# tmuird/VAEUNET

Hardware: AMD Instinct MI355X
Metric: images/sec (whole node) at 3x512x512 bs=8/GPU; Dice parity vs CPU ref (higher is better)
Workload: dtype bf16; 1 GPU; UNet(3,2) train step (fwd+CombinedLoss+bwd+clip+AdamW), random-init weights; image=3x512x512, batch_per_gpu=8, global_batch=8, parallelism=dp1, execution=hipgraph-replay, wgrad_side_stream=False

## Files before the change

### include/vaeunet.h

```cpp
#ifndef VAEUNET_H
#define VAEUNET_H
#include <stdint.h>
#ifdef __cplusplus
extern "C" {
#endif

typedef struct VuGather {
  const void* src[3];
  int64_t stride[3];
  int32_t cend[3];
  int32_t nsrc;
  int32_t C;
  int32_t N, H, W;
  int32_t Hs, Ws;
  int32_t R, S;
  int32_t sy, sx, dy, dx, oy, ox;
} VuGather;

typedef struct VuGemmFwd {
  VuGather a;
  const void* b;
  int64_t ldb;
  int32_t ncol;
  int32_t out_mode;
// ... 216 lines not shown
                    int dtype, void* stream);
int vu_attn_gate_fwd(const float* q, const float* st, const void* x,
                     int64_t xs, int64_t P, int C, float* pmap, void* out,
                     int64_t os, int dtype, void* stream);
int vu_attn_gate_bwd(const void* dout, int64_t dos, const void* x, int64_t xs,
                     const float* pmap, int64_t P, int C, void* dx,
                     int64_t dxs, float* dqpre, int dtype, void* stream);
int64_t vu_attn_psi_bwd_workspace_bytes(int64_t P, int F);
int vu_attn_psi_bwd(const void* ug, const void* ux, int64_t P, int F,
                    const float* sg, const float* tg, const float* sx,
                    const float* tx, const float* wpsi, const float* dq,
                    void* ds, float* dwpsi, float* dbpsi, int accumulate,
                    float* workspace, int dtype, void* stream);
int64_t vu_attn_psi_bwd_blocks(int64_t P);
int vu_attn_psi_bwd_bnb_ok(int F);
int vu_attn_psi_bwd_bnb(const void* ug, const void* ux, int64_t P, int F,
                        const float* sg, const float* tg, const float* sx,
                        const float* tx, const float* wpsi, const float* dq,
                        void* ds, float* dwpsi, float* dbpsi, int accumulate,
                        float* workspace, const float* mean_g, const float* invstd_g,
                        const float* mean_x, const float* invstd_x, float* bnb_g,
                        float* bnb_x, int dtype, void* stream);

int vu_pointwise_fwd(const void* x, int64_t xs, int64_t P, int C, int J,
                     const float* w, const float* b, float* y, int64_t ys,
                     int dtype, void* stream);
int64_t vu_pointwise_bwd_workspace_bytes(int64_t P, int C, int J);
int vu_pointwise_bwd(const void* x, int64_t xs, const float* dy, int64_t dys,
                     int64_t P, int C, int J, const float* w, void* dx,
                     int64_t dxs, float* dw, float* db, int accumulate,
                     float* workspace, int dtype, void* stream);
int vu_pointwise_bn_fwd(const void* x, int64_t xs, int64_t P, int C, int J,
                        const float* bn_scale, const float* bn_shift, const float* w,
                        const float* b, float* y, int64_t ys, int dtype, void* stream);
int64_t vu_pointwise_bn_bwd_blocks(int64_t P);
int vu_pointwise_bn_bwd(const void* x, int64_t xs, const float* bn_coef, int64_t coef_stride,
                        const float* dy, int64_t dys, int64_t P, int C, int J, const float* w,
                        void* dx, int64_t dxs, float* dw, float* db, int accumulate,
                        float* workspace, float* bnb, int dtype, void* stream);

int64_t vu_loss_workspace_bytes(void);
int vu_bce_dice_fwd2(const float* logits, const float* target, int64_t n,
                     double* sums, float smooth, float w_bce, float w_dice,
                     float* loss, float* parts, double* workspace,
                     void* stream);
int vu_bce_dice_fwd(const float* logits, const float* target, int64_t n,
// ... 197 lines not shown
```

### vaeunet_amd/_lib.py

```python
import ctypes as C
import os

import torch

_HERE = os.path.dirname(os.path.abspath(__file__))
LIB_PATH = os.path.join(_HERE, "libvaeunet_hip.so")
if os.environ.get("VU_LIB_PATH"):
    LIB_PATH = os.environ["VU_LIB_PATH"]

F32, BF16 = 0, 1

_p = C.c_void_p
_i = C.c_int
_l = C.c_int64
_f = C.c_float


class VuGather(C.Structure):
    _fields_ = [("src", _p * 3), ("stride", _l * 3), ("cend", C.c_int32 * 3),
                ("nsrc", C.c_int32), ("C", C.c_int32),
                ("N", C.c_int32), ("H", C.c_int32), ("W", C.c_int32),
                ("Hs", C.c_int32), ("Ws", C.c_int32), ("R", C.c_int32), ("S", C.c_int32),
                ("sy", C.c_int32), ("sx", C.c_int32), ("dy", C.c_int32), ("dx", C.c_int32),
                ("oy", C.c_int32), ("ox", C.c_int32)]
# ... 108 lines not shown
    "vu_chan_sum": (_i, [_p, _l, _i, _i, _i, _i, _i, _i, _i, _i, _p, _i, _p, _i, _p]),
    "vu_copy": (_i, [_p, _l, _i, _p, _l, _i, _l, _i, _i, _p]),
    "vu_zero": (_i, [_p, _l, _l, _i, _i, _p]),
    "vu_gpu_delay": (_i, [_i, _p]),
    "vu_zero_insert2": (_i, [_p, _l, _i, _i, _i, _i, _p, _l, _i, _i, _i, _p]),
    "vu_input_pack": (_i, [_p, _l, _l, _l, _l, _i, _i, _i, _i, _i, _p, _i, _p]),
    "vu_maxpool2_fwd": (_i, [_p, _l, _i, _i, _i, _i, _p, _l, _i, _p]),
    "vu_maxpool2_bwd": (_i, [_p, _l, _p, _l, _i, _i, _i, _i, _p, _l, _p, _l, _i, _p]),
    "vu_bn_apply_maxpool2": (_i, [_p, _l, _p, _l, _p, _l, _i, _i, _i, _i, _p, _p, _i, _i, _p]),
    "vu_upsample_fwd": (_i, [_p, _l, _i, _i, _i, _i, _p, _l, _i, _i, _i, _i, _i, _i, _i, _p]),
    "vu_upsample_bwd": (_i, [_p, _l, _i, _i, _i, _i, _p, _l, _i, _i, _i, _i, _i, _i, _i, _i,
                             _p]),
    "vu_attn_tile_rows": (_l, []),
    "vu_attn_psi_fwd": (_i, [_p, _p, _l, _i, _p, _p, _p, _p, _p, _p, _p, _p, _p, _l, _i, _p]),
    "vu_attn_gate_fwd": (_i, [_p, _p, _p, _l, _l, _i, _p, _p, _l, _i, _p]),
    "vu_attn_gate_bwd": (_i, [_p, _l, _p, _l, _p, _l, _i, _p, _l, _p, _i, _p]),
    "vu_attn_psi_bwd_workspace_bytes": (_l, [_l, _i]),
    "vu_attn_psi_bwd_blocks": (_l, [_l]),
    "vu_attn_psi_bwd_bnb_ok": (_i, [_i]),
    "vu_attn_psi_bwd_bnb": (_i, [_p, _p, _l, _i, _p, _p, _p, _p, _p, _p, _p, _p, _p, _i, _p, _p, _p, _p, _p, _p, _p,
                                 _i, _p]),
    "vu_attn_psi_bwd": (_i, [_p, _p, _l, _i, _p, _p, _p, _p, _p, _p, _p, _p, _p, _i, _p, _i,
                             _p]),
    "vu_pointwise_fwd": (_i, [_p, _l, _l, _i, _i, _p, _p, _p, _l, _i, _p]),
    "vu_pointwise_bwd_workspace_bytes": (_l, [_l, _i, _i]),
    "vu_pointwise_bn_fwd": (_i, [_p, _l, _l, _i, _i, _p, _p, _p, _p, _p, _l, _i, _p]),
    "vu_pointwise_bn_bwd_blocks": (_l, [_l]),
    "vu_pointwise_bn_bwd": (_i, [_p, _l, _p, _l, _p, _l, _l, _i, _i, _p, _p, _l, _p, _p, _i, _p, _p, _i, _p]),
    "vu_pointwise_bwd": (_i, [_p, _l, _p, _l, _l, _i, _i, _p, _p, _l, _p, _p, _i, _p, _i, _p]),
    "vu_loss_workspace_bytes": (_l, []),
    "vu_bce_dice_fwd2": (_i, [_p, _p, _l, _p, _f, _f, _f, _p, _p, _p, _p]),
    "vu_bce_dice_bwd": (_i, [_p, _p, _l, _p, _f, _f, _f, _p, _p, _p]),
    "vu_kl_free_bits2": (_i, [_p, _p, _i, _i, _f, _p, _p, _p, _p, _p]),
    "vu_sumsq": (_i, [_p, _l, _p, _p, _p]),
    "vu_dice_score": (_i, [_p, _p, _l, _f, _p, _p, _p, _p]),
    "vu_seg_counts_workspace_bytes": (_l, [_l]),
    "vu_seg_counts": (_i, [_p, _i, C.POINTER(_l), _i, _i, _p, _i, C.POINTER(_l), _i, _i, _i, _i, _i, _i, _p, _i, _p,
                           _p, _p]),
    "vu_seg_metrics": (_i, [_p, _i, _i, C.c_double, _p, _p, _i, _p, _p]),
    "vu_mt_chunk_elems": (_l, []),
    "vu_mt_grad_norm": (_i, [_p, _i, _l, _f, _p, _p, _p, _p]),
    "vu_mt_scale_grads": (_i, [_p, _i, _l, _p, _p]),
    "vu_mt_adamw": (_i, [_p, _i, _l, _f, _f, _f, _f, _f, _p, _p]),
    "vu_mt_adamw_dev": (_i, [_p, _i, _l, C.c_double, C.c_double, C.c_double, C.c_double, C.c_double, _p, _i,
                             _p]),
    "vu_mt_adamw_dev_scaled": (_i, [_p, _i, _l, C.c_double, C.c_double, C.c_double, C.c_double, C.c_double, _p,
# ... 77 lines not shown
```

### vaeunet_amd/csrc/attention.hip

```cpp
#include "host.h"

namespace {

constexpr int TILE = 256;

template <int CTRL>
VU_DEV float dpp_f(float v) {
  return __int_as_float(__builtin_amdgcn_update_dpp(0, __float_as_int(v), CTRL, 0xf, 0xf, false));
}

VU_DEV void vec8_tie(Vec8<bf16_t>& v) { asm volatile("" : "+v"(v.v)); }
VU_DEV void vec8_tie(Vec8<float>& v) { asm volatile("" : "+v"(v.a), "+v"(v.b)); }

VU_DEV float group_sum(float v, int lpp) {
  if (lpp >= 2) v += dpp_f<0xB1>(v);
  if (lpp >= 4) v += dpp_f<0x4E>(v);
  if (lpp >= 8) v += dpp_f<0x141>(v);
  if (lpp >= 16) v += dpp_f<0x140>(v);
  if (lpp >= 32) v += __shfl_xor(v, 16, 64);
  if (lpp >= 64) v += __shfl_xor(v, 32, 64);
  return v;
}

template <typename T>
// ... 85 lines not shown
    wsg[k] = sg[c + k]; wtg[k] = tg[c + k]; wsx[k] = sx[c + k]; wtx[k] = tx[c + k]; wp[k] = wpsi[c + k];
  }
  const float b = bpsi[0];
  const int niter = lpp;
  for (int it = 0; it < niter; it += U) {
    Vec8<T> va[U], vb[U];
#pragma unroll
    for (int u = 0; u < U; ++u) {
      if (it + u < niter) {
        int64_t p = p0 + w * ppw + slot + (it + u) * 4 * ppw;
        p = p < P ? p : P - 1;
        va[u].load(ug + p * F + c);
        vb[u].load(ux + p * F + c);
      }
    }
#pragma unroll
    for (int u = 0; u < U; ++u) {
      if (it + u >= niter) break;
      const int i = w * ppw + slot + (it + u) * 4 * ppw;
      const int64_t p = p0 + i;
      float acc = 0.f;
#pragma unroll
      for (int k = 0; k < 8; ++k) {
        float s = fmaxf(va[u].get(k) * wsg[k] + wtg[k] + vb[u].get(k) * wsx[k] + wtx[k], 0.f);
        acc += wp[k] * s;
      }
      if (p >= P) acc = 0.f;
      acc = group_sum(acc, lpp) + b;
      if (sub == 0) {
        sq[i] = p < P ? acc : 0.f;
        if (p < P) q[p] = acc;
      }
    }
  }
  __syncthreads();
  int64_t nvalid = P - p0 < TILE ? P - p0 : TILE;
  float v = threadIdx.x < nvalid ? sq[threadIdx.x] : 0.f;
  float tot = block_sum(v, red);
  float mean = tot / (float)nvalid;
  float d = threadIdx.x < nvalid ? sq[threadIdx.x] - mean : 0.f;
  float m2 = block_sum(d * d, red);
  if (threadIdx.x == 0) { psum[blockIdx.x] = tot; pm2[blockIdx.x] = m2; }
}

template <typename T, int U>
__global__ __launch_bounds__(256) void gate_fwd_u_kernel(const float* q, const float* st, const T* x, int64_t xs,
                                                         int64_t P, int vsh, float* pmap, T* out, int64_t os) {
// ... 50 lines not shown
template <typename T>
__global__ void gate_bwd_kernel(const T* dout, int64_t dos, const T* x, int64_t xs, const float* pmap, int64_t P,
                                int C, T* dx, int64_t dxs, float* dbnq) {
  const int lpp = C >> 3 > 64 ? 64 : C >> 3;
  const int ppw = 64 / lpp;
  const int lane = threadIdx.x & 63;
  const int sub = lane % lpp, slot = lane / lpp;
  const int64_t wave = ((int64_t)blockIdx.x * blockDim.x + threadIdx.x) >> 6;
  const int64_t nwaves = ((int64_t)gridDim.x * blockDim.x) >> 6;
  for (int64_t pb = wave * ppw; pb < P; pb += nwaves * ppw) {
    int64_t p = pb + slot;
    float acc = 0.f;
    if (p < P) {
      float pv = pmap[p];
      for (int c = sub * 8; c < C; c += lpp * 8) {
        Vec8<T> vd, vx, vo;
        vd.load(dout + p * dos + c);
        vx.load(x + p * xs + c);
#pragma unroll
        for (int k = 0; k < 8; ++k) {
          acc += vd.get(k) * vx.get(k);
          vo.set(k, vd.get(k) * pv);
        }
        vo.store(dx + p * dxs + c);
      }
    }
    acc = group_sum(acc, lpp);
    if (sub == 0 && p < P) { float pv = pmap[p]; dbnq[p] = acc * pv * (1.f - pv); }
  }
}

template <typename T, int U>
__global__ __launch_bounds__(256) void gate_bwd_u_kernel(const T* dout, int64_t dos, const T* x, int64_t xs,
                                                         const float* pmap, int64_t P, int C, T* dx, int64_t dxs,
                                                         float* dbnq) {
  const int lpp = C >> 3;
  const int ppw = 64 / lpp;
  const int lane = threadIdx.x & 63;
  const int sub = lane % lpp, slot = lane / lpp;
  const int c = sub * 8;
  const int64_t wave = ((int64_t)blockIdx.x * blockDim.x + threadIdx.x) >> 6;
  const int64_t nwaves = ((int64_t)gridDim.x * blockDim.x) >> 6;
  for (int64_t pb = wave * ppw * U; pb < P; pb += nwaves * ppw * U) {
    Vec8<T> vd[U], vx[U];
    float pv[U];
#pragma unroll
    for (int u = 0; u < U; ++u) {
      int64_t p = pb + u * ppw + slot;
      p = p < P ? p : P - 1;
      pv[u] = pmap[p];
      vd[u].load(dout + p * dos + c);
      vx[u].load(x + p * xs + c);
    }
#pragma unroll
    for (int u = 0; u < U; ++u) {
      const int64_t p = pb + u * ppw + slot;
      float acc = 0.f;
      Vec8<T> vo;
#pragma unroll
      for (int k = 0; k < 8; ++k) {
        acc += vd[u].get(k) * vx[u].get(k);
        vo.set(k, vd[u].get(k) * pv[u]);
      }
      if (p < P) vo.store(dx + p * dxs + c);
      acc = group_sum(acc, lpp);
      if (sub == 0 && p < P) dbnq[p] = acc * pv[u] * (1.f - pv[u]);
    }
  }
}

constexpr int MAXB = 1024;

template <typename T, int U, bool BNB = false>
__global__ __launch_bounds__(256) void psi_bwd_u_kernel(const T* ug, const T* ux, int64_t P, int F, const float* sg,
                                                        const float* tg, const float* sx, const float* tx,
                                                        const float* wpsi, const float* dq, T* ds, float* part,
                                                        const float* mg = nullptr, const float* ig = nullptr,
                                                        const float* mx = nullptr, const float* ix = nullptr,
                                                        float* bnb_g = nullptr, float* bnb_x = nullptr) {
  __shared__ float sh[256 * 8];
  __shared__ float sb[256];
  const int lpp = F >> 3, ppw = 64 / lpp;
  const int lane = threadIdx.x & 63, w = threadIdx.x >> 6;
  const int sub = lane % lpp, slot = lane / lpp;
  const int c = sub * 8;
  float wsg[8], wtg[8], wsx[8], wtx[8], wp[8], dw[8];
#pragma unroll
  for (int k = 0; k < 8; ++k) {
    wsg[k] = sg[c + k]; wtg[k] = tg[c + k]; wsx[k] = sx[c + k]; wtx[k] = tx[c + k]; wp[k] = wpsi[c + k];
    dw[k] = 0.f;
  }
  float bmg[8], big[8], bmx[8], bix[8], z0[8], zg[8], zx[8];
  if constexpr (BNB)
#pragma unroll
    for (int k = 0; k < 8; ++k) {
      bmg[k] = mg[c + k]; big[k] = ig[c + k]; bmx[k] = mx[c + k]; bix[k] = ix[c + k];
// ... 4 lines not shown
  for (int64_t p0 = (int64_t)blockIdx.x * TILE; p0 < P; p0 += (int64_t)gridDim.x * TILE) {
    for (int it = 0; it < niter; it += U) {
      Vec8<T> va[U], vb[U];
      float g[U];
#pragma unroll
      for (int u = 0; u < U; ++u) {
        if (it + u < niter) {
          int64_t p = p0 + w * ppw + slot + (it + u) * 4 * ppw;
          p = p < P ? p : P - 1;
          g[u] = dq[p];
          va[u].load(ug + p * F + c);
          vb[u].load(ux + p * F + c);
        }
      }
      Vec8<T> o[U];
      bool okp[U];
#pragma unroll
      for (int u = 0; u < U; ++u) {
        const int64_t p = p0 + w * ppw + slot + (it + u) * 4 * ppw;
        okp[u] = it + u < niter && p < P;
        if (okp[u] && sub == 0) db += g[u];
#pragma unroll
        for (int k = 0; k < 8; ++k) {
          float s = va[u].get(k) * wsg[k] + wtg[k] + vb[u].get(k) * wsx[k] + wtx[k];
          bool on = s > 0.f;
          if (okp[u]) dw[k] += on ? g[u] * s : 0.f;
          o[u].set(k, on ? g[u] * wp[k] : 0.f);
          if constexpr (BNB) {
            if (okp[u]) {
              const float dz = o[u].get(k);
              z0[k] += dz;
              zg[k] += dz * ((va[u].get(k) - bmg[k]) * big[k]);
              zx[k] += dz * ((vb[u].get(k) - bmx[k]) * bix[k]);
            }
          }
        }
        vec8_tie(o[u]);
      }
#pragma unroll
      for (int u = 0; u < U; ++u)
        if (okp[u]) o[u].store(ds + (p0 + w * ppw + slot + (it + u) * 4 * ppw) * F + c);
    }
  }
#pragma unroll
  for (int k = 0; k < 8; ++k) sh[threadIdx.x * 8 + k] = dw[k];
  sb[threadIdx.x] = db;
  __syncthreads();
  for (int cc = threadIdx.x; cc < F; cc += 256) {
    int sb_ = cc >> 3, k = cc & 7;
    float s = 0.f;
    s = lds_sum(sh + sb_ * 8 + k, (256 - sb_ + lpp - 1) / lpp, lpp * 8);
    part[(int64_t)blockIdx.x * (F + 1) + cc] = s;
  }
  if (threadIdx.x == 0) {
    float s = 0.f;
    s = lds_sum(sb, 256, 1);
    part[(int64_t)blockIdx.x * (F + 1) + F] = s;
  }
  if constexpr (BNB) {
    for (int q = 0; q < 3; ++q) {
      __syncthreads();
#pragma unroll
      for (int k = 0; k < 8; ++k) sh[threadIdx.x * 8 + k] = q == 0 ? z0[k] : (q == 1 ? zg[k] : zx[k]);
      __syncthreads();
// ... 296 lines not shown
extern "C" int vu_attn_gate_fwd(const float* q, const float* st_, const void* x, int64_t xs, int64_t P, int C,
                                float* pmap, void* out, int64_t os, int dtype, void* stream) {
  if (C % 8 != 0 || xs % 8 != 0 || os % 8 != 0) return (int)hipErrorInvalidValue;
  hipStream_t st = (hipStream_t)stream;
  if (P == 0) return 0;
  const int V = C / 8;
  DISPATCH_T(dtype, {
    if (tune(VU_TUNE_ATTN) && pow2(V))
      hipLaunchKernelGGL((gate_fwd_u_kernel<T, 4>), dim3(ew_grid(P * V / 4)), dim3(256), 0, st, q, st_, (const T*)x,
                         xs, P, __builtin_ctz(V), pmap, (T*)out, os);
    else
      hipLaunchKernelGGL((gate_fwd_kernel<T>), dim3(ew_grid(P * C / 8)), dim3(256), 0, st, q, st_, (const T*)x, xs, P,
                         C, pmap, (T*)out, os);
  })
  return (int)hipGetLastError();
}

extern "C" int vu_attn_gate_bwd(const void* dout, int64_t dos, const void* x, int64_t xs, const float* pmap,
                                int64_t P, int C, void* dx, int64_t dxs, float* dqpre, int dtype, void* stream) {
  if (C % 8 != 0 || !pow2(C / 8 > 64 ? 64 : C / 8) || dos % 8 || xs % 8 || dxs % 8) return (int)hipErrorInvalidValue;
  hipStream_t st = (hipStream_t)stream;
  if (P == 0) return 0;
  DISPATCH_T(dtype, {
    if (tune(VU_TUNE_ATTN) && C <= 512)
      hipLaunchKernelGGL((gate_bwd_u_kernel<T, 2>), dim3(ew_grid(P * 8)), dim3(256), 0, st, (const T*)dout, dos,
                         (const T*)x, xs, pmap, P, C, (T*)dx, dxs, dqpre);
    else
      hipLaunchKernelGGL((gate_bwd_kernel<T>), dim3(ew_grid(P * 8)), dim3(256), 0, st, (const T*)dout, dos,
                         (const T*)x, xs, pmap, P, C, (T*)dx, dxs, dqpre);
  })
  return (int)hipGetLastError();
}

extern "C" int64_t vu_attn_psi_bwd_blocks(int64_t P) {
  const int64_t nb = (P + TILE - 1) / TILE;
  return nb < MAXB ? nb : MAXB;
}

extern "C" int vu_attn_psi_bwd_bnb_ok(int F) {
  return F % 8 == 0 && pow2(F / 8) && F / 8 <= 64 && F <= 2048 && tune(VU_TUNE_ATTN) ? 1 : 0;
}

extern "C" int vu_attn_psi_bwd_bnb(const void* ug, const void* ux, int64_t P, int F, const float* sg, const float* tg,
                                   const float* sx, const float* tx, const float* wpsi, const float* dq, void* ds,
                                   float* dwpsi, float* dbpsi, int accumulate, float* workspace,
                                   const float* mean_g, const float* invstd_g, const float* mean_x,
                                   const float* invstd_x, float* bnb_g, float* bnb_x, int dtype, void* stream) {
  if (F % 8 != 0 || !pow2(F / 8) || F / 8 > 64 || F > 2048 || !tune(VU_TUNE_ATTN) || !mean_g || !invstd_g || !mean_x ||
      !invstd_x || !bnb_g || !bnb_x)
    return (int)hipErrorInvalidValue;
  const int nblk = (int)vu_attn_psi_bwd_blocks(P);
  if (nblk == 0) return 0;
  hipStream_t st = (hipStream_t)stream;
  DISPATCH_T(dtype, {
    hipLaunchKernelGGL((psi_bwd_u_kernel<T, 4, true>), dim3(nblk), dim3(256), 0, st, (const T*)ug, (const T*)ux, P, F,
                       sg, tg, sx, tx, wpsi, dq, (T*)ds, workspace, mean_g, invstd_g, mean_x, invstd_x, bnb_g, bnb_x);
  })
  hipLaunchKernelGGL(part_final, dim3((F + 1 + 31) / 32), dim3(COLSUM_THREADS), 0, st, workspace, nblk, F + 1, dwpsi,
                     F, dbpsi, accumulate);
  return (int)hipGetLastError();
}

extern "C" int64_t vu_attn_psi_bwd_workspace_bytes(int64_t P, int F) {
  int64_t nb = (P + TILE - 1) / TILE;
  return (nb < MAXB ? nb : MAXB) * (F + 1) * (int64_t)sizeof(float);
}

extern "C" int vu_attn_psi_bwd(const void* ug, const void* ux, int64_t P, int F, const float* sg, const float* tg,
                               const float* sx, const float* tx, const float* wpsi, const float* dq, void* ds,
                               float* dwpsi, float* dbpsi, int accumulate, float* workspace, int dtype,
                               void* stream) {
  if (F % 8 != 0 || !pow2(F / 8) || F / 8 > 64 || F > 2048) return (int)hipErrorInvalidValue;
  int nblk = (int)((P + TILE - 1) / TILE);
  if (nblk == 0) return 0;
  if (nblk > MAXB) nblk = MAXB;
  hipStream_t st = (hipStream_t)stream;
  DISPATCH_T(dtype, {
    if (tune(VU_TUNE_ATTN))
      hipLaunchKernelGGL((psi_bwd_u_kernel<T, 4>), dim3(nblk), dim3(256), 0, st, (const T*)ug, (const T*)ux, P, F, sg,
// ... 101 lines not shown
```

### vaeunet_amd/engine.py

```python
import warnings

import torch

from . import kernels as K
from ._lib import BF16, F32


OVERLAP_WGRAD = False

FUSE_BN_BWD_REDUCE = True


class SideStream:

    _per_device = {}

    def __init__(self, device):
        self.stream = torch.cuda.Stream(device=device)
        self.keep = []
        self.pending = False

    @classmethod
    def get(cls, device):
        key = torch.device(device).index
# ... 449 lines not shown

def down_fwd(M, mod, x, pend=None, defer=False):
    seq = mod.maxpool_conv[1].double_conv
    if x is None:
        y, coef = pend
        N, C_, H, W = y.shape
        x = M.act(N, C_, H, W)
        xp = M.act(N, C_, H // 2, W // 2)
        K.bn_apply_maxpool(y, x, xp, coef, True, M.d)
    else:
        xp = K.maxpool_fwd(x, M.d)
    out, sdc = double_conv_fwd(M, seq, [xp], defer=defer)
    return x, out, (x, sdc)


def down_bwd(M, mod, saved, dout, add=None):
    x, sdc = saved
    seq = mod.maxpool_conv[1].double_conv
    dxp = double_conv_bwd(M, seq, sdc, dout, True)
    return PoolGrad(dxp, add, x)


FUSE_ATTN_BN_REDUCE = True


def attention_fwd(M, att, g, x):
    N, _, H, W = x.shape
    P = N * H * W
    wg, bng = att.W_g[0], att.W_g[1]
    wx, bnx = att.W_x[0], att.W_x[1]
    wp, bnp = att.psi[0], att.psi[1]
    F = wg.out_channels
    ug = M.act(N, F, H, W)
    stg = K.gemm_fwd(K.gather1x1([g]), w1x1_fwd(wg.weight, M.d), F, ug, M.d, bias=wg.bias,
                     stats=bng.training)
    ux = M.act(N, F, H, W)
    stx = K.gemm_fwd(K.gather1x1([x]), w1x1_fwd(wx.weight, M.d), F, ux, M.d, bias=wx.bias,
                     stats=bnx.training)
    cg = bn_coef(bng, stg, F)
    cx = bn_coef(bnx, stx, F)
    tile = K.query("vu_attn_tile_rows")
    tiles = (P + tile - 1) // tile
    q = torch.empty((N, 1, H, W), dtype=torch.float32, device=x.device)
    psum = torch.empty(tiles, dtype=torch.float32, device=x.device)
    pm2 = torch.empty_like(psum)
    K.call("vu_attn_psi_fwd", K.ptr(ug), K.ptr(ux), P, F, K.ptr(cg[0]), K.ptr(cg[1]), K.ptr(cx[0]),
# ... 4 lines not shown
    out = M.act(N, x.shape[1], H, W)
    K.call("vu_attn_gate_fwd", K.ptr(q), K.ptr(cq), K.ptr(x), K.pstride(x), P, x.shape[1],
           K.ptr(pmap), K.ptr(out), K.pstride(out), M.d, K.stream())
    _fire_psi_hooks(att.psi, pmap)
    return out, (g, x, ug, ux, cg, cx, q, cq, pmap)


def _fire_psi_hooks(psi, pmap):
    if psi._forward_hooks:
        for hook in list(psi._forward_hooks.values()):
            hook(psi, (None,), pmap)


def attention_bwd(M, att, saved, dout, dg_out, dg_acc):
    g, x, ug, ux, cg, cx, q, cq, pmap = saved
    N, _, H, W = x.shape
    P = N * H * W
    wg, bng = att.W_g[0], att.W_g[1]
    wx, bnx = att.W_x[0], att.W_x[1]
    wp, bnp = att.psi[0], att.psi[1]
    F = wg.out_channels
    dx = torch.empty_like(x)
    dbnq = torch.empty((N, 1, H, W), dtype=torch.float32, device=x.device)
    K.call("vu_attn_gate_bwd", K.ptr(dout), K.pstride(dout), K.ptr(x), K.pstride(x), K.ptr(pmap),
           P, x.shape[1], K.ptr(dx), K.pstride(dx), K.ptr(dbnq), M.d, K.stream())
    gw, accw = grad_sink(bnp.weight)
    gb, _ = grad_sink(bnp.bias)
    dq = torch.empty_like(q)
    K.bn_backward(dbnq, q, cq, bnp.weight, False, gw, gb, accw, dq, F32, train=bnp.training)
    ds = M.act(N, F, H, W)
    gwp, accp = grad_sink(wp.weight)
    gbp, _ = grad_sink(wp.bias)
    ws = K.workspace_f32(K.query("vu_attn_psi_bwd_workspace_bytes", P, F), x.device)
    pg = px = None
    if FUSE_ATTN_BN_REDUCE and K.query("vu_attn_psi_bwd_bnb_ok", F):
        nb = K.query("vu_attn_psi_bwd_blocks", P)
        bg = torch.empty((nb, 2, F), dtype=torch.float32, device=x.device)
        bx = torch.empty_like(bg)
        K.call("vu_attn_psi_bwd_bnb", K.ptr(ug), K.ptr(ux), P, F, K.ptr(cg[0]), K.ptr(cg[1]),
               K.ptr(cx[0]), K.ptr(cx[1]), K.ptr(wp.weight), K.ptr(dq), K.ptr(ds), K.ptr(gwp),
               K.ptr(gbp), 1 if accp else 0, K.ptr(ws), K.ptr(cg[2]), K.ptr(cg[3]), K.ptr(cx[2]),
               K.ptr(cx[3]), K.ptr(bg), K.ptr(bx), M.d, K.stream())
        pg, px = K.BnbPart(bg, nb, ug), K.BnbPart(bx, nb, ux)
    else:
        K.call("vu_attn_psi_bwd", K.ptr(ug), K.ptr(ux), P, F, K.ptr(cg[0]), K.ptr(cg[1]),
               K.ptr(cx[0]), K.ptr(cx[1]), K.ptr(wp.weight), K.ptr(dq), K.ptr(ds), K.ptr(gwp),
               K.ptr(gbp), 1 if accp else 0, K.ptr(ws), M.d, K.stream())
    if pg is not None:
        dug, dux = bn_bwd_pair(ds, (ug, cg, bng, pg), (ux, cx, bnx, px), M)
    else:
        dug = bn_bwd(ds, ug, cg, bng, False, M)
        dux = bn_bwd(ds, ux, cx, bnx, False, M)

    def wgs():
        wgrad1x1(dug, [g], wg.weight, M)
        bias_grad(dug, wg.bias, M, bn=bng)
        wgrad1x1(dux, [x], wx.weight, M)
        bias_grad(dux, wx.bias, M, bn=bnx)
        M.notify([wg.weight, wg.bias, wx.weight, wx.bias, wp.weight, wp.bias, bng.weight, bng.bias,
                  bnx.weight, bnx.bias, bnp.weight, bnp.bias])
    M.side(wgs, dug, dux, g, x)
    if dg_out is not None:
        dst, coff = dg_out
        K.gemm_fwd(K.gather1x1([dug]), w1x1_dgrad(wg.weight, M.d), g.shape[1], dst, M.d,
                   out_coff=coff, accumulate=dg_acc)
    K.gemm_fwd(K.gather1x1([dux]), w1x1_dgrad(wx.weight, M.d), x.shape[1], dx, M.d, accumulate=True)
    return dx


def up_fwd(M, mod, x1, x2, defer_out=False):
    N, _, H, W = x2.shape
    h, w = x1.shape[2], x1.shape[3]
    bilinear = isinstance(mod.up, torch.nn.Upsample)
    uh, uw = 2 * h, 2 * w
    dy_, dx_ = H - uh, W - uw
    py, px = dy_ // 2, dx_ // 2
    crop = dy_ < 0 or dx_ < 0
    if bilinear:
        cu = x1.shape[1]
        u = M.act(N, cu, H, W)
        K.upsample_fwd(x1, u, uh, uw, py, px, M.d)
    else:
        cu = mod.up.out_channels
        if crop:
# ... 107 lines not shown
```

### vaeunet_amd/kernels.py

```python
import ctypes as C

import torch

from . import _lib
from ._lib import ptr, call, query, stream, VuGather, VuGemmFwd, VuGemmWgrad

CL = torch.channels_last


def dcode(dtype):
    if dtype == torch.bfloat16:
        return _lib.BF16
    if dtype == torch.float32:
        return _lib.F32
    raise TypeError(f"unsupported activation dtype {dtype}")


def empty_act(N, Cc, H, W, dtype, device):
    return torch.empty((N, Cc, H, W), dtype=dtype, device=device, memory_format=CL)


def zeros_act(N, Cc, H, W, dtype, device):
    y = torch.empty((N, Cc, H, W), dtype=dtype, device=device, memory_format=CL)
    zero(y)
# ... 103 lines not shown


def _gemm_tag(g, kind):
    if g.R == 3 and g.C >= 16:
        return f"conv3x3_{kind}"
    if g.R == 3:
        return f"conv3x3_image_{kind}"
    if g.R == 2:
        return f"convT_{kind}"
    return f"gemm1x1_{kind}"


class Stats:

    def __init__(self, psum, pm2, tiles, tile_rows, rows):
        self.psum, self.pm2, self.tiles, self.tile_rows, self.rows = psum, pm2, tiles, tile_rows, rows
        self.minmax = None


class BnbPart:

    def __init__(self, part, nblk, x):
        self.part, self.nblk, self.x = part, nblk, x


def gemm_fwd(g, wmat, ncol, out, dtype, out_coff=0, bias=None, stats=False, accumulate=False,
             convT=None, kind="fwd", strided=None, bnb=None, flops=None, relu=False, zbias=None):
    a = VuGemmFwd()
    a.a = g
    a.b = wmat.data_ptr()
    a.ldb = wmat.shape[-1] if wmat.dim() == 2 else wmat.stride(0)
    a.ncol = ncol
    a.out = out.data_ptr()
    a.out_stride = pstride(out)
    a.out_coff = out_coff
    if convT is not None:
        a.out_mode = 1
        a.oH, a.oW, a.opy, a.opx, a.cout = convT
    elif strided is not None:
        a.out_mode = 2
        a.oH, a.oW, a.opy, a.opx = strided
        a.cout = ncol
    else:
        a.out_mode = 0
    a.bias = bias.data_ptr() if bias is not None else None
    a.zbias = zbias.data_ptr() if zbias is not None else None
# ... 433 lines not shown
```

Baseline: 540.4 images/sec.

## Fuse attention-gate backward tail into one kernel with MFMA dgrad GEMMs

Result: faster. 550.1 images/sec (median of 6 runs) (+1.8%).

```diff
diff --git a/include/vaeunet.h b/include/vaeunet.h
--- a/include/vaeunet.h
+++ b/include/vaeunet.h
@@ -262,6 +262,17 @@
                         const float* mean_x, const float* invstd_x, float* bnb_g,
                         float* bnb_x, int dtype, void* stream);
 
+int64_t vu_attn_tail_bwd_tile(int F, int C);
+int vu_attn_tail_bwd_ok(int64_t P, int F, int C, int64_t ldg, int64_t ldx, int64_t dos,
+                        int64_t dgs, int64_t dg_coff, int64_t dxs, int dtype);
+int vu_attn_tail_bwd(const void* ug, const void* ux, const float* dq, int64_t P, int F, int C,
+                     const float* sg, const float* tg, const float* sx, const float* tx,
+                     const float* wpsi, const float* mean_g, const float* coef_g,
+                     const float* mean_x, const float* coef_x, const void* wdg, int64_t ldg,
+                     const void* wdx, int64_t ldx, const void* dout, int64_t dos,
+                     const float* pmap, void* dg, int64_t dgs, int64_t dg_coff, int dg_acc,
+                     void* dx, int64_t dxs, void* dug, void* dux, int dtype, void* stream);
+
 int vu_pointwise_fwd(const void* x, int64_t xs, int64_t P, int C, int J,
                      const float* w, const float* b, float* y, int64_t ys,
                      int dtype, void* stream);
diff --git a/vaeunet_amd/_lib.py b/vaeunet_amd/_lib.py
--- a/vaeunet_amd/_lib.py
+++ b/vaeunet_amd/_lib.py
@@ -154,6 +154,10 @@
                                  _i, _p]),
     "vu_attn_psi_bwd": (_i, [_p, _p, _l, _i, _p, _p, _p, _p, _p, _p, _p, _p, _p, _i, _p, _i,
                              _p]),
+    "vu_attn_tail_bwd_tile": (_l, [_i, _i]),
+    "vu_attn_tail_bwd_ok": (_i, [_l, _i, _i, _l, _l, _l, _l, _l, _l, _i]),
+    "vu_attn_tail_bwd": (_i, [_p, _p, _p, _l, _i, _i, _p, _p, _p, _p, _p, _p, _p, _p, _p, _p, _l, _p, _l, _p, _l,
+                              _p, _p, _l, _l, _i, _p, _l, _p, _p, _i, _p]),
     "vu_pointwise_fwd": (_i, [_p, _l, _l, _i, _i, _p, _p, _p, _l, _i, _p]),
     "vu_pointwise_bwd_workspace_bytes": (_l, [_l, _i, _i]),
     "vu_pointwise_bn_fwd": (_i, [_p, _l, _l, _i, _i, _p, _p, _p, _p, _p, _l, _i, _p]),
diff --git a/vaeunet_amd/csrc/attention.hip b/vaeunet_amd/csrc/attention.hip
--- a/vaeunet_amd/csrc/attention.hip
+++ b/vaeunet_amd/csrc/attention.hip
@@ -1,4 +1,5 @@
 #include "host.h"
+#include "attn_pre.h"
 
 namespace {
 
@@ -131,7 +132,7 @@
       float acc = 0.f;
 #pragma unroll
       for (int k = 0; k < 8; ++k) {
-        float s = fmaxf(va[u].get(k) * wsg[k] + wtg[k] + vb[u].get(k) * wsx[k] + wtx[k], 0.f);
+        float s = fmaxf(attn_pre(va[u].get(k), wsg[k], wtg[k], vb[u].get(k), wsx[k], wtx[k]), 0.f);
         acc += wp[k] * s;
       }
       if (p >= P) acc = 0.f;
@@ -228,7 +229,7 @@
           acc += vd.get(k) * vx.get(k);
           vo.set(k, vd.get(k) * pv);
         }
-        vo.store(dx + p * dxs + c);
+        if (dx) vo.store(dx + p * dxs + c);
       }
     }
     acc = group_sum(acc, lpp);
@@ -236,7 +237,7 @@
   }
 }
 
-template <typename T, int U>
+template <typename T, int U, bool DX = true>
 __global__ __launch_bounds__(256) void gate_bwd_u_kernel(const T* dout, int64_t dos, const T* x, int64_t xs,
                                                          const float* pmap, int64_t P, int C, T* dx, int64_t dxs,
                                                          float* dbnq) {
@@ -266,9 +267,10 @@
 #pragma unroll
       for (int k = 0; k < 8; ++k) {
         acc += vd[u].get(k) * vx[u].get(k);
-        vo.set(k, vd[u].get(k) * pv[u]);
-      }
-      if (p < P) vo.store(dx + p * dxs + c);
+        if constexpr (DX) vo.set(k, vd[u].get(k) * pv[u]);
+      }
+      if constexpr (DX)
+        if (p < P) vo.store(dx + p * dxs + c);
       acc = group_sum(acc, lpp);
       if (sub == 0 && p < P) dbnq[p] = acc * pv[u] * (1.f - pv[u]);
     }
@@ -277,7 +279,7 @@
 
 constexpr int MAXB = 1024;
 
-template <typename T, int U, bool BNB = false>
+template <typename T, int U, bool BNB = false, bool DS = true>
 __global__ __launch_bounds__(256) void psi_bwd_u_kernel(const T* ug, const T* ux, int64_t P, int F, const float* sg,
                                                         const float* tg, const float* sx, const float* tx,
                                                         const float* wpsi, const float* dq, T* ds, float* part,
@@ -328,7 +330,7 @@
         if (okp[u] && sub == 0) db += g[u];
 #pragma unroll
         for (int k = 0; k < 8; ++k) {
-          float s = va[u].get(k) * wsg[k] + wtg[k] + vb[u].get(k) * wsx[k] + wtx[k];
+          float s = attn_pre(va[u].get(k), wsg[k], wtg[k], vb[u].get(k), wsx[k], wtx[k]);
           bool on = s > 0.f;
           if (okp[u]) dw[k] += on ? g[u] * s : 0.f;
           o[u].set(k, on ? g[u] * wp[k] : 0.f);
@@ -343,9 +345,10 @@
         }
         vec8_tie(o[u]);
       }
-#pragma unroll
-      for (int u = 0; u < U; ++u)
-        if (okp[u]) o[u].store(ds + (p0 + w * ppw + slot + (it + u) * 4 * ppw) * F + c);
+      if constexpr (DS)
+#pragma unroll
+        for (int u = 0; u < U; ++u)
+          if (okp[u]) o[u].store(ds + (p0 + w * ppw + slot + (it + u) * 4 * ppw) * F + c);
     }
   }
 #pragma unroll
@@ -688,9 +691,12 @@
   hipStream_t st = (hipStream_t)stream;
   if (P == 0) return 0;
   DISPATCH_T(dtype, {
-    if (tune(VU_TUNE_ATTN) && C <= 512)
+    if (tune(VU_TUNE_ATTN) && C <= 512 && dx)
       hipLaunchKernelGGL((gate_bwd_u_kernel<T, 2>), dim3(ew_grid(P * 8)), dim3(256), 0, st, (const T*)dout, dos,
                          (const T*)x, xs, pmap, P, C, (T*)dx, dxs, dqpre);
+    else if (tune(VU_TUNE_ATTN) && C <= 512)
+      hipLaunchKernelGGL((gate_bwd_u_kernel<T, 2, false>), dim3(ew_grid(P * 8)), dim3(256), 0, st, (const T*)dout,
+                         dos, (const T*)x, xs, pmap, P, C, (T*)nullptr, dxs, dqpre);
     else
       hipLaunchKernelGGL((gate_bwd_kernel<T>), dim3(ew_grid(P * 8)), dim3(256), 0, st, (const T*)dout, dos,
                          (const T*)x, xs, pmap, P, C, (T*)dx, dxs, dqpre);
@@ -719,8 +725,14 @@
   if (nblk == 0) return 0;
   hipStream_t st = (hipStream_t)stream;
   DISPATCH_T(dtype, {
-    hipLaunchKernelGGL((psi_bwd_u_kernel<T, 4, true>), dim3(nblk), dim3(256), 0, st, (const T*)ug, (const T*)ux, P, F,
-                       sg, tg, sx, tx, wpsi, dq, (T*)ds, workspace, mean_g, invstd_g, mean_x, invstd_x, bnb_g, bnb_x);
+    if (ds)
+      hipLaunchKernelGGL((psi_bwd_u_kernel<T, 4, true>), dim3(nblk), dim3(256), 0, st, (const T*)ug, (const T*)ux, P,
+                         F, sg, tg, sx, tx, wpsi, dq, (T*)ds, workspace, mean_g, invstd_g, mean_x, invstd_x, bnb_g,
+                         bnb_x);
+    else
+      hipLaunchKernelGGL((psi_bwd_u_kernel<T, 4, true, false>), dim3(nblk), dim3(256), 0, st, (const T*)ug,
+                         (const T*)ux, P, F, sg, tg, sx, tx, wpsi, dq, (T*)nullptr, workspace, mean_g, invstd_g,
+                         mean_x, invstd_x, bnb_g, bnb_x);
   })
   hipLaunchKernelGGL(part_final, dim3((F + 1 + 31) / 32), dim3(COLSUM_THREADS), 0, st, workspace, nblk, F + 1, dwpsi,
                      F, dbpsi, accumulate);
diff --git a/vaeunet_amd/csrc/attention_tail.hip b/vaeunet_amd/csrc/attention_tail.hip
--- /dev/null
+++ b/vaeunet_amd/csrc/attention_tail.hip
@@ -0,0 +1,325 @@
+#include <type_traits>
+
+#include "host.h"
+#include "attn_pre.h"
+
+namespace {
+
+VU_DEV uint32_t pack2(float a, float b) { return (uint32_t)f2bf(a) | ((uint32_t)f2bf(b) << 16); }
+
+enum { Q_SG, Q_TG, Q_SX, Q_TX, Q_WP, Q_MG, Q_AG, Q_BG, Q_EG, Q_MX, Q_AX, Q_BX, Q_EX, NQ };
+
+struct AttnTail {
+  const bf16_t *ug, *ux;
+  const float *dq, *pmap;
+  const float* coef[NQ];
+  const bf16_t *wg, *wx;
+  int64_t ldg, ldx;
+  const bf16_t* dout;
+  int64_t dos;
+  bf16_t* dg;
+  int64_t dgs;
+  int dg_acc;
+  bf16_t* dx;
+  int64_t dxs;
+  bf16_t *dug, *dux;
+  int64_t P;
+};
+
+template <int KS, int NJ, int NF, int NW>
+__global__ __launch_bounds__(64 * NW, NW == 4 ? 2 : 1) void attn_tail_kernel(AttnTail p) {
+  constexpr int K = 32 * KS, N = 16 * NJ, PX = 16 * NF, NT = 64 * NW;
+  constexpr int GS = 4;
+  static_assert(NJ % GS == 0, "whole 64-column groups");
+  __shared__ __attribute__((aligned(16))) char wsm[2][N * K * 2];
+  __shared__ __attribute__((aligned(16))) float csm[NQ][K];
+
+  const int ntiles = (int)(p.P / PX);
+  const int lane = threadIdx.x & 63;
+  const int wid = __builtin_amdgcn_readfirstlane(threadIdx.x >> 6);
+  const int gq = lane >> 4, r16 = lane & 15;
+
+  auto wrow = [&](int j, int r) { return (j / GS) * 16 * GS + 4 * GS * (r >> 2) + 4 * (j % GS) + (r & 3); };
+  {
+    constexpr int PIECES = NJ * KS * 64;
+#pragma unroll
+    for (int img = 0; img < 2; ++img) {
+      const bf16_t* bmat = img ? p.wx : p.wg;
+      const int64_t ld = img ? p.ldx : p.ldg;
+      for (int e = threadIdx.x; e < PIECES; e += NT) {
+        const int l = e & 63, jk = e >> 6, j = jk / KS, ks = jk - j * KS;
+        *reinterpret_cast<u32x4*>(wsm[img] + e * 16) =
+            *reinterpret_cast<const u32x4*>(bmat + (int64_t)wrow(j, l & 15) * ld + 32 * ks + 8 * (l >> 4));
+      }
+    }
+#pragma unroll
+    for (int q = 0; q < NQ; ++q)
+      for (int c = threadIdx.x; c < K; c += NT) csm[q][c] = p.coef[q][c];
+    __syncthreads();
+  }
+
+  const int tstride = gridDim.x * NW;
+  auto tile_px = [&](int t) {
+    asm volatile("" : "+s"(t));
+    return (int64_t)t * PX;
+  };
+  auto opq = [](uint32_t v) {
+    asm volatile("" : "+v"(v));
+    return v;
+  };
+  const uint32_t lk0 = (uint32_t)(r16 * K + 8 * gq);
+  auto load = [&](int t, u32x4 (&a)[NF][KS], u32x4 (&b)[NF][KS], float (&g)[NF], float (&pv)[NF]) {
+    const int64_t pb = tile_px(t);
+    const uint32_t lk = opq(lk0), lr = opq((uint32_t)r16);
+    const bf16_t *ugb = p.ug + pb * K + lk, *uxb = p.ux + pb * K + lk;
+    const float *dqb = p.dq + pb + lr, *pmb = p.pmap + pb + lr;
+#pragma unroll
+    for (int f = 0; f < NF; ++f) {
+      g[f] = dqb[16 * f];
+      pv[f] = pmb[16 * f];
+#pragma unroll
+      for (int ks = 0; ks < KS; ++ks) {
+        a[f][ks] = *reinterpret_cast<const u32x4*>(ugb + 16 * f * K + 32 * ks);
+        b[f][ks] = *reinterpret_cast<const u32x4*>(uxb + 16 * f * K + 32 * ks);
+      }
+    }
+  };
+  u32x4 na[NF][KS], nb[NF][KS];
+  float ng[NF], npv[NF];
+  int tile = blockIdx.x * NW + wid;
+  if (tile < ntiles) load(tile, na, nb, ng, npv);
+  for (; tile < ntiles; tile += tstride) {
+    const int64_t pb = tile_px(tile);
+    int lo = 0;
+    asm volatile("" : "+v"(lo));
+    auto coef8 = [&](int q, int ks, float (&d)[8]) {
+      const char* s = reinterpret_cast<const char*>(&csm[q][32 * ks + 8 * gq]) + lo;
+      const f32x4 u = *reinterpret_cast<const f32x4*>(s), v = *reinterpret_cast<const f32x4*>(s + 16);
+#pragma unroll
+      for (int k = 0; k < 4; ++k) { d[k] = u[k]; d[4 + k] = v[k]; }
+    };
+    u32x4 ag[NF][KS], ax[NF][KS];
+    float pv[NF];
+#pragma unroll
+    for (int f = 0; f < NF; ++f) pv[f] = npv[f];
+#pragma unroll
+    for (int ks = 0; ks < KS; ++ks) {
+      Vec8<bf16_t> va[NF], vb[NF];
+      float dsv[NF][8];
+      {
+        float wsg[8], wtg[8], wsx[8], wtx[8], wp[8];
+        coef8(Q_SG, ks, wsg); coef8(Q_TG, ks, wtg); coef8(Q_SX, ks, wsx); coef8(Q_TX, ks, wtx); coef8(Q_WP, ks, wp);
+#pragma unroll
+        for (int f = 0; f < NF; ++f) {
+          va[f].v = na[f][ks];
+          vb[f].v = nb[f][ks];
+#pragma unroll
+          for (int k = 0; k < 8; ++k) {
+            float s = attn_pre(va[f].get(k), wsg[k], wtg[k], vb[f].get(k), wsx[k], wtx[k]);
+            bool on = s > 0.f;
+            float gw = rnd<bf16_t>(ng[f] * wp[k]);
+            asm volatile("" : "+v"(gw));
+            dsv[f][k] = on ? gw : 0.f;
+          }
+        }
+        __builtin_amdgcn_sched_barrier(0);
+      }
+#pragma unroll
+      for (int side = 0; side < 2; ++side) {
+        float mu[8], a[8], b[8], e[8];
+        coef8(side ? Q_MX : Q_MG, ks, mu); coef8(side ? Q_AX : Q_AG, ks, a);
+        coef8(side ? Q_BX : Q_BG, ks, b); coef8(side ? Q_EX : Q_EG, ks, e);
+#pragma unroll
+        for (int f = 0; f < NF; ++f) {
+          const Vec8<bf16_t>& vx = side ? vb[f] : va[f];
+          Vec8<bf16_t> o;
+          o.zero();
+#pragma unroll
+          for (int k = 0; k < 8; ++k) {
+            const float dz = dsv[f][k];
+            o.set(k, fmaf(a[k], dz, b[k] * (vx.get(k) - mu[k])) + e[k]);
+          }
+          asm volatile("" : "+v"(o.v));
+          (side ? ax : ag)[f][ks] = o.v;
+        }
+        __builtin_amdgcn_sched_barrier(0);
+      }
+    }
+    if (tile + tstride < ntiles) load(tile + tstride, na, nb, ng, npv);
+    {
+      const uint32_t lk = opq(lk0);
+      bf16_t *dugb = p.dug + pb * K + lk, *duxb = p.dux + pb * K + lk;
+#pragma unroll
+      for (int f = 0; f < NF; ++f)
+#pragma unroll
+        for (int ks = 0; ks < KS; ++ks) {
+          *reinterpret_cast<u32x4*>(dugb + 16 * f * K + 32 * ks) = ag[f][ks];
+          *reinterpret_cast<u32x4*>(duxb + 16 * f * K + 32 * ks) = ax[f][ks];
+        }
+    }
+
+    auto add_old = [&](u32x4& v, const u32x4 o) {
+#pragma unroll
+      for (int w = 0; w < 4; ++w)
+        v[w] = pack2(__uint_as_float(o[w] << 16) + __uint_as_float(v[w] << 16),
+                     __uint_as_float(o[w] & 0xffff0000u) + __uint_as_float(v[w] & 0xffff0000u));
+    };
+    auto gemm = [&](const char* wimg, const u32x4 (&pf)[NF][KS], bf16_t* out, int64_t os, auto old_tag) {
+      constexpr int OLD = decltype(old_tag)::value;
+      f32x4 acc[NF][NJ];
+#pragma unroll
+      for (int f = 0; f < NF; ++f)
+#pragma unroll
+        for (int j = 0; j < NJ; ++j) acc[f][j] = f32x4{0, 0, 0, 0};
+#pragma unroll
+      for (int ks = 0; ks < KS; ++ks)
+#pragma unroll
+        for (int j = 0; j < NJ; ++j) {
+          const u32x4 wf = *reinterpret_cast<const u32x4*>(wimg + lo + ((j * KS + ks) * 64 + lane) * 16);
+#pragma unroll
+          for (int f = 0; f < NF; ++f)
+            acc[f][j] = __builtin_amdgcn_mfma_f32_16x16x32_bf16(__builtin_bit_cast(bf16x8, wf),
+                                                                __builtin_bit_cast(bf16x8, pf[f][ks]), acc[f][j], 0, 0, 0);
+          if constexpr (KS * NJ >= 64)
+            if ((j & 7) == 7) __builtin_amdgcn_sched_barrier(0);
+        }
+#pragma unroll
+      for (int f = 0; f < NF; ++f) {
+        const uint32_t row = (uint32_t)(16 * f + r16);
+        bf16_t* outp = out + pb * os + opq(row * (uint32_t)os + 8 * gq);
+        const bf16_t* dop = p.dout + pb * p.dos + opq(row * (uint32_t)p.dos + 8 * gq);
+        constexpr int GC = NJ / GS < 2 ? NJ / GS : 2;
+#pragma unroll
+        for (int g0 = 0; g0 < NJ / GS; g0 += GC) {
+          u32x4 c[GC][2];
+#pragma unroll
+          for (int gi = 0; gi < GC; ++gi) {
+            const int grp = g0 + gi;
+#pragma unroll
+            for (int h2 = 0; h2 < 2; ++h2) {
+              const f32x4 a = acc[f][grp * 4 + 2 * h2] + 0.f, b = acc[f][grp * 4 + 2 * h2 + 1] + 0.f;
+              c[gi][h2] = u32x4{pack2(a[0], a[1]), pack2(a[2], a[3]), pack2(b[0], b[1]), pack2(b[2], b[3])};
+            }
+#pragma unroll
+            for (int w = 0; w < 4; ++w) {
+              const auto r1 = __builtin_amdgcn_permlane16_swap(c[gi][0][w], c[gi][1][w], false, false);
+              const auto r2 = __builtin_amdgcn_permlane32_swap(r1[0], r1[1], false, false);
+              c[gi][0][w] = r2[0];
+              c[gi][1][w] = r2[1];
+            }
+          }
+          if constexpr (OLD != 0) {
+            u32x4 o[GC][2];
+#pragma unroll
+            for (int gi = 0; gi < GC; ++gi)
+#pragma unroll
+              for (int h = 0; h < 2; ++h) {
+                const int col = (g0 + gi) * 64 + 32 * h;
+                if constexpr (OLD == 1) o[gi][h] = *reinterpret_cast<const u32x4*>(outp + col);
+                else o[gi][h] = *reinterpret_cast<const u32x4*>(dop + col);
+              }
+#pragma unroll
+            for (int gi = 0; gi < GC; ++gi)
+#pragma unroll
+              for (int h = 0; h < 2; ++h) {
+                if constexpr (OLD == 2) {
+#pragma unroll
+                  for (int w = 0; w < 4; ++w)
+                    o[gi][h][w] = pack2(__uint_as_float(o[gi][h][w] << 16) * pv[f],
+                                        __uint_as_float(o[gi][h][w] & 0xffff0000u) * pv[f]);
+                }
+                add_old(c[gi][h], o[gi][h]);
+              }
+          }
+#pragma unroll
+          for (int gi = 0; gi < GC; ++gi)
+#pragma unroll
+            for (int h = 0; h < 2; ++h)
+              *reinterpret_cast<u32x4*>(outp + (g0 + gi) * 64 + 32 * h) = c[gi][h];
+        }
+      }
+    };
+    if (p.dg_acc) gemm(wsm[0], ag, p.dg, p.dgs, std::integral_constant<int, 1>{});
+    else gemm(wsm[0], ag, p.dg, p.dgs, std::integral_constant<int, 0>{});
+    gemm(wsm[1], ax, p.dx, p.dxs, std::integral_constant<int, 2>{});
+  }
+}
+
+constexpr int nf_of(int ks, int nj) {
+  return (16 / nj < 4 ? 16 / nj : 4) < (4 / ks) ? (16 / nj < 4 ? 16 / nj : 4) : 4 / ks;
+}
+constexpr int nw_of(int ks, int nj) { return 2 * (16 * nj) * (32 * ks) * 2 > 72 * 1024 ? 8 : 4; }
+
+template <int KS, int NJ>
+int launch_nj(const AttnTail& p, hipStream_t st) {
+  constexpr int NF = nf_of(KS, NJ), NW = nw_of(KS, NJ);
+  const int64_t tiles = p.P / (16 * NF);
+  int64_t nblk = (tiles + NW - 1) / NW;
+  const int64_t cap = (NW == 4 ? 2 : 1) * (int64_t)cu_count();
+  if (nblk > cap) nblk = cap;
+  if (nblk == 0) return 0;
+  hipLaunchKernelGGL((attn_tail_kernel<KS, NJ, NF, NW>), dim3((unsigned)nblk), dim3(64 * NW), 0, st, p);
+  return (int)hipGetLastError();
+}
+
+template <int KS>
+int launch_ks(const AttnTail& p, int C, hipStream_t st) {
+  switch (C / 16) {
+    case 4: return launch_nj<KS, 4>(p, st);
+    case 8: return launch_nj<KS, 8>(p, st);
+    case 16: return launch_nj<KS, 16>(p, st);
+    default: return (int)hipErrorInvalidValue;
+  }
+}
+
+}
+
+extern "C" int64_t vu_attn_tail_bwd_tile(int F, int C) {
+  if ((F != 32 && F != 64 && F != 128) || (C != 64 && C != 128 && C != 256)) return 0;
+  return 16 * nf_of(F / 32, C / 16);
+}
+
+extern "C" int vu_attn_tail_bwd_ok(int64_t P, int F, int C, int64_t ldg, int64_t ldx, int64_t dos, int64_t dgs,
+                                   int64_t dg_coff, int64_t dxs, int dtype) {
+  if (dtype != VU_BF16) return 0;
+  const int64_t px = vu_attn_tail_bwd_tile(F, C);
+  if (px == 0) return 0;
+  if (ldg % 8 != 0 || ldg < F || ldx % 8 != 0 || ldx < F) return 0;
+  if (dos % 8 != 0 || dos < C || dgs % 8 != 0 || dg_coff % 8 != 0 || dg_coff < 0 || dgs < dg_coff + C || dxs % 8 != 0 ||
+      dxs < C)
+    return 0;
+  if (dos >= (1 << 20) || dgs >= (1 << 20) || dxs >= (1 << 20)) return 0;
+  if (P <= 0 || P % px != 0 || P >= ((int64_t)1 << 31)) return 0;
+  return 1;
+}
+
+extern "C" int vu_attn_tail_bwd(const void* ug, const void* ux, const float* dq, int64_t P, int F, int C,
+                                const float* sg, const float* tg, const float* sx, const float* tx,
+                                const float* wpsi, const float* mean_g, const float* coef_g, const float* mean_x,
+                                const float* coef_x, const void* wdg, int64_t ldg, const void* wdx, int64_t ldx,
+                                const void* dout, int64_t dos, const float* pmap, void* dg, int64_t dgs,
+                                int64_t dg_coff, int dg_acc, void* dx, int64_t dxs, void* dug, void* dux, int dtype,
+                                void* stream) {
+  if (!vu_attn_tail_bwd_ok(P, F, C, ldg, ldx, dos, dgs, dg_coff, dxs, dtype)) return (int)hipErrorInvalidValue;
+  if (!ug || !ux || !dq || !sg || !tg || !sx || !tx || !wpsi || !mean_g || !coef_g || !mean_x || !coef_x || !wdg ||
+      !wdx || !dout || !pmap || !dg || !dx || !dug || !dux)
+    return (int)hipErrorInvalidValue;
+  AttnTail p;
+  p.ug = (const bf16_t*)ug; p.ux = (const bf16_t*)ux; p.dq = dq; p.pmap = pmap;
+  p.coef[Q_SG] = sg; p.coef[Q_TG] = tg; p.coef[Q_SX] = sx; p.coef[Q_TX] = tx; p.coef[Q_WP] = wpsi;
+  p.coef[Q_MG] = mean_g; p.coef[Q_AG] = coef_g; p.coef[Q_BG] = coef_g + F; p.coef[Q_EG] = coef_g + 2 * F;
+  p.coef[Q_MX] = mean_x; p.coef[Q_AX] = coef_x; p.coef[Q_BX] = coef_x + F; p.coef[Q_EX] = coef_x + 2 * F;
+  p.wg = (const bf16_t*)wdg; p.wx = (const bf16_t*)wdx; p.ldg = ldg; p.ldx = ldx;
+  p.dout = (const bf16_t*)dout; p.dos = dos;
+  p.dg = (bf16_t*)dg + dg_coff; p.dgs = dgs; p.dg_acc = dg_acc;
+  p.dx = (bf16_t*)dx; p.dxs = dxs;
+  p.dug = (bf16_t*)dug; p.dux = (bf16_t*)dux;
+  p.P = P;
+  hipStream_t st = (hipStream_t)stream;
+  switch (F) {
+    case 32: return launch_ks<1>(p, C, st);
+    case 64: return launch_ks<2>(p, C, st);
+    case 128: return launch_ks<4>(p, C, st);
+    default: return (int)hipErrorInvalidValue;
+  }
+}
diff --git a/vaeunet_amd/csrc/attn_pre.h b/vaeunet_amd/csrc/attn_pre.h
--- /dev/null
+++ b/vaeunet_amd/csrc/attn_pre.h
@@ -0,0 +1,7 @@
+#pragma once
+#include "common.h"
+
+VU_DEV float attn_pre(float a, float wsg, float wtg, float b, float wsx, float wtx) {
+#pragma clang fp contract(off)
+  return a * wsg + wtg + b * wsx + wtx;
+}
diff --git a/vaeunet_amd/engine.py b/vaeunet_amd/engine.py
--- a/vaeunet_amd/engine.py
+++ b/vaeunet_amd/engine.py
@@ -495,6 +495,20 @@
 
 
 FUSE_ATTN_BN_REDUCE = True
+FUSE_ATTN_TAIL = True
+ATTN_TAIL_MIN_TILES_PER_CU = 8
+
+
+def _attn_tail_ok(M, P, F, g, x, dout, dg_out, wdg, wdx, dx):
+    if not FUSE_ATTN_TAIL or M.d != BF16 or dg_out is None or g.shape[1] != x.shape[1]:
+        return False
+    C_ = x.shape[1]
+    dst, coff = dg_out
+    if not K.query("vu_attn_tail_bwd_ok", P, F, C_, wdg.shape[-1], wdx.shape[-1], K.pstride(dout),
+                   K.pstride(dst), coff, K.pstride(dx), M.d):
+        return False
+    cus = torch.cuda.get_device_properties(x.device).multi_processor_count
+    return P // K.query("vu_attn_tail_bwd_tile", F, C_) >= ATTN_TAIL_MIN_TILES_PER_CU * cus
 
 
 def attention_fwd(M, att, g, x):
@@ -545,31 +559,55 @@
     F = wg.out_channels
     dx = torch.empty_like(x)
     dbnq = torch.empty((N, 1, H, W), dtype=torch.float32, device=x.device)
+    bnb = FUSE_ATTN_BN_REDUCE and K.query("vu_attn_psi_bwd_bnb_ok", F)
+    tail = bool(bnb) and _attn_tail_ok(M, P, F, g, x, dout, dg_out, w1x1_dgrad(wg.weight, M.d),
+                                       w1x1_dgrad(wx.weight, M.d), dx)
     K.call("vu_attn_gate_bwd", K.ptr(dout), K.pstride(dout), K.ptr(x), K.pstride(x), K.ptr(pmap),
-           P, x.shape[1], K.ptr(dx), K.pstride(dx), K.ptr(dbnq), M.d, K.stream())
+           P, x.shape[1], None if tail else K.ptr(dx), K.pstride(dx), K.ptr(dbnq), M.d, K.stream())
     gw, accw = grad_sink(bnp.weight)
     gb, _ = grad_sink(bnp.bias)
     dq = torch.empty_like(q)
     K.bn_backward(dbnq, q, cq, bnp.weight, False, gw, gb, accw, dq, F32, train=bnp.training)
-    ds = M.act(N, F, H, W)
+    ds = None if tail else M.act(N, F, H, W)
     gwp, accp = grad_sink(wp.weight)
     gbp, _ = grad_sink(wp.bias)
     ws = K.workspace_f32(K.query("vu_attn_psi_bwd_workspace_bytes", P, F), x.device)
     pg = px = None
-    if FUSE_ATTN_BN_REDUCE and K.query("vu_attn_psi_bwd_bnb_ok", F):
+    if bnb:
         nb = K.query("vu_attn_psi_bwd_blocks", P)
         bg = torch.empty((nb, 2, F), dtype=torch.float32, device=x.device)
         bx = torch.empty_like(bg)
         K.call("vu_attn_psi_bwd_bnb", K.ptr(ug), K.ptr(ux), P, F, K.ptr(cg[0]), K.ptr(cg[1]),
-               K.ptr(cx[0]), K.ptr(cx[1]), K.ptr(wp.weight), K.ptr(dq), K.ptr(ds), K.ptr(gwp),
-               K.ptr(gbp), 1 if accp else 0, K.ptr(ws), K.ptr(cg[2]), K.ptr(cg[3]), K.ptr(cx[2]),
+               K.ptr(cx[0]), K.ptr(cx[1]), K.ptr(wp.weight), K.ptr(dq), None if tail else K.ptr(ds),
+               K.ptr(gwp), K.ptr(gbp), 1 if accp else 0, K.ptr(ws), K.ptr(cg[2]), K.ptr(cg[3]), K.ptr(cx[2]),
                K.ptr(cx[3]), K.ptr(bg), K.ptr(bx), M.d, K.stream())
         pg, px = K.BnbPart(bg, nb, ug), K.BnbPart(bx, nb, ux)
     else:
         K.call("vu_attn_psi_bwd", K.ptr(ug), K.ptr(ux), P, F, K.ptr(cg[0]), K.ptr(cg[1]),
                K.ptr(cx[0]), K.ptr(cx[1]), K.ptr(wp.weight), K.ptr(dq), K.ptr(ds), K.ptr(gwp),
                K.ptr(gbp), 1 if accp else 0, K.ptr(ws), M.d, K.stream())
-    if pg is not None:
+    if tail:
+        ks = []
+        for u_, c_, bn_, part in ((ug, cg, bng, pg), (ux, cx, bnx, px)):
+            gw_, gb_, acc_ = bn_grad_sinks(bn_)
+            ks.append(K.bn_backward_finish(part, u_, c_, bn_.weight, gw_, gb_, acc_, train=bn_.training))
+        dug, dux = torch.empty_like(ug), torch.empty_like(ux)
+        wdg, wdx = w1x1_dgrad(wg.weight, M.d), w1x1_dgrad(wx.weight, M.d)
+        dst, coff = dg_out
+
+        def run_tail():
+            K.call("vu_attn_tail_bwd", K.ptr(ug), K.ptr(ux), K.ptr(dq), P, F, x.shape[1], K.ptr(cg[0]),
+                   K.ptr(cg[1]), K.ptr(cx[0]), K.ptr(cx[1]), K.ptr(wp.weight), K.ptr(cg[2]), K.ptr(ks[0]),
+                   K.ptr(cx[2]), K.ptr(ks[1]), K.ptr(wdg), wdg.shape[-1], K.ptr(wdx), wdx.shape[-1],
+                   K.ptr(dout), K.pstride(dout), K.ptr(pmap), K.ptr(dst), K.pstride(dst), coff,
+                   1 if dg_acc else 0, K.ptr(dx), K.pstride(dx), K.ptr(dug), K.ptr(dux), M.d, K.stream())
+        if K.AUDIT is None:
+            run_tail()
+        else:
+            dx.copy_(dout.float() * pmap)
+            K.audited_gemm(K.gather1x1([dug]), wdg, g.shape[1], dst, M.d, coff, dg_acc,
+                           lambda: K.audited_gemm(K.gather1x1([dux]), wdx, x.shape[1], dx, M.d, 0, True, run_tail))
+    elif pg is not None:
         dug, dux = bn_bwd_pair(ds, (ug, cg, bng, pg), (ux, cx, bnx, px), M)
     else:
         dug = bn_bwd(ds, ug, cg, bng, False, M)
@@ -583,6 +621,8 @@
         M.notify([wg.weight, wg.bias, wx.weight, wx.bias, wp.weight, wp.bias, bng.weight, bng.bias,
                   bnx.weight, bnx.bias, bnp.weight, bnp.bias])
     M.side(wgs, dug, dux, g, x)
+    if tail:
+        return dx
     if dg_out is not None:
         dst, coff = dg_out
         K.gemm_fwd(K.gather1x1([dug]), w1x1_dgrad(wg.weight, M.d), g.shape[1], dst, M.d,
diff --git a/vaeunet_amd/kernels.py b/vaeunet_amd/kernels.py
--- a/vaeunet_amd/kernels.py
+++ b/vaeunet_amd/kernels.py
@@ -149,6 +149,22 @@
 
     def __init__(self, part, nblk, x):
         self.part, self.nblk, self.x = part, nblk, x
+
+
+def audited_gemm(g, wmat, ncol, out, dtype, out_coff, accumulate, launch):
+    if AUDIT is None:
+        return launch()
+    a = VuGemmFwd()
+    a.a = g
+    a.b = wmat.data_ptr()
+    a.ldb = wmat.shape[-1] if wmat.dim() == 2 else wmat.stride(0)
+    a.ncol = ncol
+    a.out = out.data_ptr()
+    a.out_stride = pstride(out)
+    a.out_coff = out_coff
+    a.out_mode = 0
+    a.accumulate = 1 if accumulate else 0
+    return AUDIT.gemm_fwd(a, dtype, g, wmat, out, None, None, launch)
 
 
 def gemm_fwd(g, wmat, ncol, out, dtype, out_coff=0, bias=None, stats=False, accumulate=False,
```
